# arnfred/Fast-Match

Measured on AMD Instinct MI355X. Metric: descriptor-pair distances/sec (cross-checked 1-NN + ratio test at 0.7), higher is better.
Workload: dtype int8

## Files before the change

fast-match_amd/csrc/filter6.hip:

```cpp
#include "tile_ops.h"
#include "fp6_filter.h"
#include "fp6_plan.h"

namespace fm {

typedef int   v8i_6  __attribute__((ext_vector_type(8)));
typedef int   v2i_6  __attribute__((ext_vector_type(2)));
typedef float v4f_6  __attribute__((ext_vector_type(4)));
typedef float v16f_6 __attribute__((ext_vector_type(16)));

#define F6_LDS_PTR(p) ((__attribute__((address_space(3))) void*)(p))
#define F6_GLB_PTR(p) ((const __attribute__((address_space(1))) void*)(p))
#define F6_INLINE __attribute__((always_inline))

constexpr int kF6NC = 4, kF6NW = 8;
constexpr int kF6PieceRows = 512;
constexpr int kF6ChunkRows = 32 * kF6NC * kF6NW;
constexpr int kF6Units = kStageRows / kTileRows;
constexpr float kF6Never = 3.0e38f;
constexpr int kF6HitSlots = 128;
static_assert(kF6HitSlots >= 64 && kF6HitSlots % 64 == 0, "a block's ballot must fit an empty list; the flush copies 64 at a time");
static_assert(3 * kStageBytes + kF6NW * kF6HitSlots * 8 <= 65536, "the kernel's static LDS");

struct F6Params {
    const uint8_t* col_rows6;
    const int32_t* col_stat;
    int            ncols;
    int            ncols_pad;
    const uint8_t* red_rows6;
    const float*   red_aux6;
    const int32_t* red_max;
    int            nstages, nsplit, nchunks, stages_per_split, ncols_alloc;
    int            nsplit_f, stages_per_split_f;
    unsigned long long* partial;
    const unsigned* cut;
    uint2*         rec;
    unsigned       cap;
    unsigned*      cnt;
    const int8_t*  col_rows8;
    const int32_t* col_norm;
    const int8_t*  red_rows8;
    const int32_t* red_norm;
    int            nred;
};

struct F6Batch {
    F6Params p[kRRBatchMax];
    int      n;
    int      first_block[kRRBatchMax + 1];
};

__device__ __forceinline__ void f6_issue_stage(const uint8_t* red_rows6, const float* red_aux6, int stage, char* buf, int wave, int lane)
{
    const uint8_t* src_rows = red_rows6 + (size_t)stage * kStageRowBytes;
    const int slot = lane & 7;
    constexpr int kPieces = 16 / kF6NW;
#pragma unroll
    for (int i = 0; i < kPieces; ++i) {
        const int g   = wave * kPieces + i;
        const int row = g * 8 + (lane >> 3);
        const uint8_t* src = src_rows + (unsigned)(row * kDim + 16 * (slot ^ ((row >> 1) & 7)));
        __builtin_amdgcn_global_load_lds(F6_GLB_PTR(src), F6_LDS_PTR(buf + g * 1024), 16, 0, 0);
    }
    if (wave == kF6NW - 1) {
        const float* src = red_aux6 + (size_t)stage * (kStageAuxBytes / 4) + (unsigned)(lane * 4);
        __builtin_amdgcn_global_load_lds(F6_GLB_PTR(src), F6_LDS_PTR(buf + kStageRowBytes), 16, 0, 0);
    }
}

struct F6Unit {
    v8i_6  a[2];
    v16f_6 c;
};

__device__ __forceinline__ float f6_max16(const v16f_6& a)
{
    const float m0 = fmaxf(fmaxf(a[0], a[1]), a[2]);
    const float m1 = fmaxf(fmaxf(a[3], a[4]), a[5]);
    const float m2 = fmaxf(fmaxf(a[6], a[7]), a[8]);
    const float m3 = fmaxf(fmaxf(a[9], a[10]), a[11]);
    const float m4 = fmaxf(fmaxf(a[12], a[13]), a[14]);
    const float m5 = fmaxf(fmaxf(m0, m1), m2);
    const float m6 = fmaxf(fmaxf(m3, m4), a[15]);
    return fmaxf(m5, m6);
}

__global__ __launch_bounds__(64 * kF6NW, 2)
void filter6_kernel(F6Batch b)
{
    __shared__ __attribute__((aligned(16))) char smem[3 * kStageBytes + kF6NW * kF6HitSlots * 8];
    int pair = 0;
#pragma unroll
    for (int i = 1; i < kRRBatchMax; ++i) pair += (int)blockIdx.x >= b.first_block[i] ? 1 : 0;
    const F6Params& p = b.p[pair];
    const int bid = (int)blockIdx.x - b.first_block[pair];

    const int tid  = threadIdx.x;
    const int lane = tid & 63;
    const int wave = tid >> 6;
    const int r32  = lane & 31;
    const int hs   = lane >> 5;
    const int nsplit = p.nsplit_f, nstages = p.nstages, per = p.stages_per_split_f, ncols = p.ncols, ncols_pad = p.ncols_pad;
    const int ncols_alloc = p.ncols_alloc;
    const int nch = (p.nchunks + 1) >> 1;
    const uint8_t* const red_rows6 = p.red_rows6;
    const float* const red_aux6 = p.red_aux6;
    uint2* const rec = p.rec;
    unsigned* const cnt = p.cnt;
    const unsigned cap = p.cap;
    const int split = __builtin_amdgcn_readfirstlane(bid / nch), chunk = bid - split * nch;
    if (split >= nsplit) return;
    const int st0 = split * per;
    const int st1 = min(st0 + per, nstages);
    const int cb  = chunk * kF6ChunkRows + wave * (32 * kF6NC);

    const unsigned dstar = *p.cut;
    if (dstar == kNoRatioCut) {
        if (tid == 0) cnt[1] = 1u;
        return;
    }
    {
        const int nslices = p.nsplit;
        const bool second = chunk * kF6ChunkRows + kF6PieceRows < ncols_alloc;
        for (int s = split; s < nslices; s += nsplit) {
            unsigned long long* mine = p.partial + (size_t)s * ncols_alloc + chunk * kF6ChunkRows;
            mine[tid] = ~0ull;
            if (second) mine[kF6PieceRows + tid] = ~0ull;
        }
    }

    v8i_6 bf[kF6NC][2];
    float thr[kF6NC];
    constexpr int kDmaPerWave = 16 / kF6NW;
    {
        const int um = p.red_max[0], em = p.red_max[1];
        v4i lo[kF6NC][2], stat[kF6NC];
        v2i_6 hi[kF6NC][2];
#pragma unroll
        for (int j = 0; j < kF6NC; ++j) {
            const int n = min(cb + 32 * j + r32, ncols_pad - 1);
#pragma unroll
            for (int h = 0; h < 2; ++h) {
                const uint8_t* src = p.col_rows6 + (size_t)n * kDim + 32 * (2 * h + hs);
                asm volatile("global_load_dwordx4 %0, %1, off" : "=v"(lo[j][h]) : "v"(src) : "memory");
                asm volatile("global_load_dwordx2 %0, %1, off offset:16" : "=v"(hi[j][h]) : "v"(src) : "memory");
            }
            asm volatile("global_load_dwordx4 %0, %1, off" : "=v"(stat[j]) : "v"(p.col_stat + 4 * (size_t)n) : "memory");
        }
        const int nfirst = min(st1 - st0, 2);
        if (nfirst > 0) f6_issue_stage(red_rows6, red_aux6, st0, smem, wave, lane);
        if (nfirst > 1) f6_issue_stage(red_rows6, red_aux6, st0 + 1, smem + kStageBytes, wave, lane);
        if (nfirst > 1) {
            if (wave == kF6NW - 1) asm volatile("s_waitcnt vmcnt(%0)" :: "n"(2 * (kDmaPerWave + 1)) : "memory");
            else                   asm volatile("s_waitcnt vmcnt(%0)" :: "n"(2 * kDmaPerWave) : "memory");
        } else {
            asm volatile("s_waitcnt vmcnt(0)" ::: "memory");
        }
#pragma unroll
        for (int j = 0; j < kF6NC; ++j)
            asm volatile("" : "+v"(lo[j][0]), "+v"(hi[j][0]), "+v"(lo[j][1]), "+v"(hi[j][1]), "+v"(stat[j]));
#pragma unroll
        for (int j = 0; j < kF6NC; ++j)
            if (cb + 32 * j + r32 >= ncols_pad) {
                lo[j][0] = lo[j][1] = v4i{0, 0, 0, 0};
                hi[j][0] = hi[j][1] = v2i_6{0, 0};
            }
#pragma unroll
        for (int j = 0; j < kF6NC; ++j) {
            const int n = cb + 32 * j + r32;
            thr[j] = n < ncols ? fp6_threshold_acc(fp6_threshold(stat[j][0], stat[j][1], stat[j][2], um, em, dstar)) : kF6Never;
#pragma unroll
            for (int h = 0; h < 2; ++h)
                bf[j][h] = v8i_6{lo[j][h][0], lo[j][h][1], lo[j][h][2], lo[j][h][3], hi[j][h][0], hi[j][h][1], 0, 0};
        }
    }

    const int sw = (r32 >> 1) & 7;
    int aoff0[2], aoff1[2];
#pragma unroll
    for (int h = 0; h < 2; ++h) {
        aoff0[h] = r32 * kDim + 16 * ((2 * (2 * h + hs)) ^ sw);
        aoff1[h] = r32 * kDim + 16 * ((2 * (2 * h + hs) + 1) ^ sw);
    }
    const int xoff = kStageRowBytes + 16 * hs;

    auto hand_over = [&](auto buf_tag, int st) F6_INLINE {
        constexpr int BUF = decltype(buf_tag)::value;
        if (st + 1 < st1) {
            if (wave == kF6NW - 1) asm volatile("s_waitcnt vmcnt(%0)" :: "n"(kDmaPerWave + 1) : "memory");
            else                   asm volatile("s_waitcnt vmcnt(%0)" :: "n"(kDmaPerWave) : "memory");
        } else {
            asm volatile("s_waitcnt vmcnt(0)" ::: "memory");
        }
        asm volatile("s_waitcnt lgkmcnt(0)\n\ts_barrier" ::: "memory");
        if (st + 2 < st1) f6_issue_stage(red_rows6, red_aux6, st + 2, smem + ((BUF + 2) % 3) * kStageBytes, wave, lane);
    };

    auto read_unit = [&](F6Unit& x, const char* buf, int u) F6_INLINE {
        const char* rows = buf + 32 * u * kDim;
#pragma unroll
        for (int h = 0; h < 2; ++h) {
            const v4i   lo = *(const v4i*)(rows + aoff0[h]);
            const v2i_6 hi = *(const v2i_6*)(rows + aoff1[h]);
            x.a[h] = __builtin_shufflevector(__builtin_shufflevector(lo, lo, 0, 1, 2, 3, -1, -1, -1, -1),
                                             __builtin_shufflevector(hi, hi, 0, 1, -1, -1, -1, -1, -1, -1), 0, 1, 2, 3, 8, 9, -1, -1);
        }
        v4f_6 c[4];
#pragma unroll
        for (int q = 0; q < 4; ++q) c[q] = *(const v4f_6*)(buf + xoff + (32 * u + 8 * q) * 4);
        x.c = v16f_6{c[0][0], c[0][1], c[0][2], c[0][3], c[1][0], c[1][1], c[1][2], c[1][3],
                     c[2][0], c[2][1], c[2][2], c[2][3], c[3][0], c[3][1], c[3][2], c[3][3]};
    };

    const uint2* const hits = (const uint2*)(smem + 3 * kStageBytes) + wave * kF6HitSlots;
    const unsigned hits_lds = (unsigned)(uintptr_t)F6_LDS_PTR(hits);
    unsigned nrec = 0;
    auto flush = [&]() F6_INLINE {
        unsigned base = 0;
        if (lane == 0) base = atomicAdd(cnt, nrec);
        base = (unsigned)__builtin_amdgcn_readfirstlane((int)base);
#pragma unroll
        for (int k = 0; k < kF6HitSlots / 64; ++k) {
            const unsigned i = (unsigned)(64 * k + lane);
            if (i < nrec) {
                const uint2 r = hits[i];
                if (base + i < cap) rec[base + i] = r;
                else                cnt[1] = 1u;
            }
        }
        asm volatile("s_waitcnt vmcnt(0)" ::: "memory");
        nrec = 0;
    };

    auto multiply = [&](const F6Unit& x, unsigned unit, F6Unit& y, const char* ybuf, auto yu_tag) F6_INLINE {
        v16f_6 acc[kF6NC];
        __builtin_amdgcn_s_setprio(2);
#pragma unroll
        for (int h = 0; h < 2; ++h)
#pragma unroll
            for (int j = 0; j < kF6NC; ++j)
                acc[j] = __builtin_amdgcn_mfma_scale_f32_32x32x64_f8f6f4(x.a[h], bf[j][h], h == 0 ? x.c : acc[j], 2, 2, 0, 0, 0, 0);
        __builtin_amdgcn_sched_barrier(0);
        if constexpr (decltype(yu_tag)::value >= 0) read_unit(y, ybuf, decltype(yu_tag)::value);
        __builtin_amdgcn_s_setprio(0);
        float tmax[kF6NC];
        bool any = false;
#pragma unroll
        for (int j = 0; j < kF6NC; ++j) {
            tmax[j] = f6_max16(acc[j]);
            any |= tmax[j] >= thr[j];
        }
        if (__builtin_amdgcn_ballot_w64(any) != 0ull) {
#pragma unroll
            for (int j = 0; j < kF6NC; ++j) {
                const bool hit = tmax[j] >= thr[j];
                const unsigned long long m = __builtin_amdgcn_ballot_w64(hit);
                if (m == 0ull) continue;
                const unsigned pc = (unsigned)__popcll(m);
                if (nrec + pc > (unsigned)kF6HitSlots) flush();
                const unsigned rank = __builtin_amdgcn_mbcnt_hi((unsigned)(m >> 32), __builtin_amdgcn_mbcnt_lo((unsigned)m, 0u));
                if (hit) {
                    const unsigned long long r = ((unsigned long long)(unit | ((unsigned)hs << 31)) << 32) | (unsigned)(cb + 32 * j + r32);
                    asm volatile("ds_write_b64 %0, %1" :: "v"(hits_lds + 8u * (nrec + rank)), "v"(r) : "memory");
                }
                nrec += pc;
            }
        }
    };

    F6Unit ua, ub;
    ub.a[0] = ub.a[1] = v8i_6{0, 0, 0, 0, 0, 0, 0, 0};
#pragma unroll
    for (int r = 0; r < 16; ++r) ub.c[r] = kFp6PadInit;
    std::integral_constant<int, 0> u0;  std::integral_constant<int, 1> u1;  std::integral_constant<int, 2> u2;
    std::integral_constant<int, 3> u3;  std::integral_constant<int, -1> none;
    auto stage = [&](auto buf_tag, int st) F6_INLINE {
        constexpr int BUF = decltype(buf_tag)::value;
        const char* buf = smem + BUF * kStageBytes;
        const unsigned unit0 = (unsigned)(st * kF6Units);
        hand_over(buf_tag, st);
        multiply(ub, unit0 - 1, ua, buf, u0);
        multiply(ua, unit0,     ub, buf, u1);
        multiply(ub, unit0 + 1, ua, buf, u2);
        multiply(ua, unit0 + 2, ub, buf, u3);
    };

    if (st0 >= st1) return;
    for (int st = st0; st < st1; st += 3) {
        stage(std::integral_constant<int, 0>{}, st);
        if (st + 1 < st1) stage(std::integral_constant<int, 1>{}, st + 1);
        if (st + 2 < st1) stage(std::integral_constant<int, 2>{}, st + 2);
    }
    multiply(ub, (unsigned)(st1 * kF6Units) - 1u, ua, smem, none);
    if (nrec != 0u) flush();
}

__global__ __launch_bounds__(256)
void rescore6_kernel(F6Batch b)
{
    const int lane = threadIdx.x & 63;
    const unsigned wave = (blockIdx.x * 256u + threadIdx.x) >> 6, nwaves = gridDim.x * 4u;
    for (int pi = 0; pi < b.n; ++pi) {
        const F6Params& p = b.p[pi];
        if (p.cnt[1] != 0u) continue;
        unsigned n = p.cnt[0];
        n = n < p.cap ? n : p.cap;
        const unsigned dstar = *p.cut;
        for (unsigned r = wave; r < n; r += nwaves) {
            const uint2 rc = p.rec[r];
            const int c = (int)rc.x;
            const int rr = lane & 15, kq = lane >> 4;
            const int m = (int)((rc.y & 0x7fffffffu) * 32u) + (rr & 3) + 8 * (rr >> 2) + 4 * (int)(rc.y >> 31);
            const int8_t* a = p.col_rows8 + (size_t)c * kDim + 32 * kq;
            const int8_t* y = p.red_rows8 + (size_t)m * kDim + 32 * kq;
            int dot = 0;
#pragma unroll
            for (int w = 0; w < 2; ++w) {
                const v4i x = *(const v4i*)(a + 16 * w);
                const v4i z = *(const v4i*)(y + 16 * w);
#pragma unroll
                for (int k = 0; k < 4; ++k) dot = __builtin_amdgcn_sdot4(x[k], z[k], dot, false);
            }
            dot += __shfl_xor(dot, 16);
            dot += __shfl_xor(dot, 32);
            const unsigned d2 = (unsigned)(p.col_norm[c] + p.red_norm[m] - 2 * dot);
            unsigned long long key = (m < p.nred && d2 < dstar) ? ((unsigned long long)d2 << 32) | (unsigned)m : ~0ull;
#pragma unroll
            for (int o = 8; o > 0; o >>= 1) {
                const unsigned long long other = __shfl_xor(key, o);
                key = other < key ? other : key;
            }
            if (lane == 0 && key != ~0ull) atomicMin(p.partial + c, key);
        }
    }
}

__global__ __launch_bounds__(256)
void prep6_kernel(const int8_t* __restrict__ rows8, int64_t n, int64_t n_pad, uint8_t* __restrict__ rows6,
                  float* __restrict__ aux6, int32_t* __restrict__ stat6, int32_t* __restrict__ max6)
{
    __shared__ uint8_t code[256];
    code[threadIdx.x] = (uint8_t)fp6_code((int)threadIdx.x);
    __syncthreads();
    const int k = threadIdx.x & 3;
    int umax = 0, emax = 0;
    for (int64_t row = (int64_t)blockIdx.x * 64 + (threadIdx.x >> 2); row < n_pad; row += (int64_t)gridDim.x * 64) {
        unsigned w[8] = {0, 0, 0, 0, 0, 0, 0, 0};
        int usq = 0, hsq = 0, esq = 0;
        if (row < n) {
            const uint4 lo = *(const uint4*)(rows8 + row * kDim + 32 * k), hi = *(const uint4*)(rows8 + row * kDim + 32 * k + 16);
            const unsigned src[8] = {lo.x, lo.y, lo.z, lo.w, hi.x, hi.y, hi.z, hi.w};
            unsigned long long bits = 0;
            int have = 0, out = 0;
#pragma unroll
            for (int i = 0; i < 32; ++i) {
                const int v = (int)(((src[i >> 2] >> (8 * (i & 3))) & 0xffu) ^ 0x80u);
                const int cd = code[v], x = fp6_value32(cd);
                usq += v * v; hsq += x * x; esq += (v - x) * (v - x);
                bits |= (unsigned long long)cd << have;
                have += 6;
                if (have >= 32) { w[out++] = (unsigned)bits; bits >>= 32; have -= 32; }
            }
        }
        *(uint4*)(rows6 + row * kDim + 32 * k)      = make_uint4(w[0], w[1], w[2], w[3]);
        *(uint4*)(rows6 + row * kDim + 32 * k + 16) = make_uint4(w[4], w[5], w[6], w[7]);
        usq += __shfl_xor(usq, 1); usq += __shfl_xor(usq, 2);
        hsq += __shfl_xor(hsq, 1); hsq += __shfl_xor(hsq, 2);
        esq += __shfl_xor(esq, 1); esq += __shfl_xor(esq, 2);
        if (k == 0) {
            *(int4*)(stat6 + 4 * row) = make_int4(usq, hsq, esq, 0);
            const int64_t st = row / kStageRows, r = row % kStageRows;
            aux6[st * 256 + r] = row < n ? fp6_acc_init(usq) : kFp6PadInit;
            aux6[st * 256 + 128 + r] = 0.f;
        }
        umax = max(umax, usq);
        emax = max(emax, esq);
    }
    for (int o = 32; o > 0; o >>= 1) {
        umax = max(umax, __shfl_xor(umax, o));
        emax = max(emax, __shfl_xor(emax, o));
    }
    if ((threadIdx.x & 63) == 0) {
        if (umax > 0) atomicMax(max6, umax);
        if (emax > 0) atomicMax(max6 + 1, emax);
    }
}

hipError_t launch_prep6(const Bank& b, int grid_max, hipStream_t stream)
{
    hipError_t e = hipMemsetAsync(b.max6, 0, 8, stream);
    if (e != hipSuccess) return e;
    int64_t grid = (b.n_pad + 63) / 64;
    if (grid_max > 0 && grid > grid_max) grid = grid_max;
    hipLaunchKernelGGL(prep6_kernel, dim3((unsigned)grid), dim3(256), 0, stream, (const int8_t*)b.rows8, b.n, b.n_pad,
                       b.rows6, b.aux6, b.stat6, b.max6);
    return hipGetLastError();
}

bool filter6_usable(const Bank& cols, const Bank& red)
{
    return cols.kind == FM_BANK_I8 && red.kind == FM_BANK_I8 && cols.dim == kDim && red.dim == kDim &&
           cols.rows6 && red.rows6 && cols.rows8 && red.rows8;
}

hipError_t launch_filter6(int n, const Bank* const* cols, const Bank* const* red, const RowReducePlan* plans,
                          unsigned long long* const* partial, const unsigned* const* cut, const Filter6Ws& ws, hipStream_t stream)
{
    if (n < 1 || n > kRRBatchMax) return hipErrorInvalidValue;
    uint2* const rec = ws.rec;  const unsigned cap = ws.cap;  unsigned* const cnt = ws.cnt;
    F6Batch b;
    long long total = 0;
    Fp6PlanPair pp[kRRBatchMax];
    for (int i = 0; i < n; ++i) pp[i] = Fp6PlanPair{(plans[i].nchunks + 1) / 2, (int)(red[i]->n_pad / kStageRows)};
    const int L = ws.nsplit == 0 ? fp6_plan_stages(pp, n, ws.resident, kFp6PlanOverhead) : 0;
    for (int i = 0; i < n; ++i) {
        const RowReducePlan& pl = plans[i];
        if (pl.nb != 4 || pl.nw != 8 || !filter6_usable(*cols[i], *red[i]) || !cut[i]) return hipErrorInvalidValue;
        F6Params& p = b.p[i];
        p.col_rows6 = cols[i]->rows6;  p.col_stat = cols[i]->stat6;  p.ncols = (int)cols[i]->n;  p.ncols_pad = (int)cols[i]->n_pad;
        p.red_rows6 = red[i]->rows6;   p.red_aux6 = red[i]->aux6;    p.red_max = red[i]->max6;
        p.nstages = (int)(red[i]->n_pad / kStageRows);
        p.nsplit = pl.nsplit;  p.nchunks = pl.nchunks;  p.stages_per_split = pl.stages_per_split;  p.ncols_alloc = pl.ncols_alloc;
        if (ws.nsplit < 0)      { p.nsplit_f = pl.nsplit;  p.stages_per_split_f = pl.stages_per_split; }
        else if (ws.nsplit > 0) fp6_plan_split_forced(p.nstages, ws.nsplit, &p.nsplit_f, &p.stages_per_split_f);
        else                    fp6_plan_split(p.nstages, L, &p.nsplit_f, &p.stages_per_split_f);
        p.partial = partial[i];  p.cut = cut[i];
        p.rec = rec + (size_t)i * cap;  p.cap = cap;  p.cnt = cnt + 2 * i;
        p.col_rows8 = cols[i]->rows8;  p.col_norm = cols[i]->norm;  p.red_rows8 = red[i]->rows8;  p.red_norm = red[i]->norm;
        p.nred = (int)red[i]->n;
        b.first_block[i] = (int)total;
        total += (long long)((pl.nchunks + 1) / 2) * p.nsplit_f;
    }
    if (total > INT32_MAX) return hipErrorInvalidValue;
    for (int i = n; i < kRRBatchMax; ++i) b.p[i] = b.p[0];
    b.first_block[n] = (int)total;
    for (int i = n + 1; i <= kRRBatchMax; ++i) b.first_block[i] = INT32_MAX;
    b.n = n;
    hipError_t e = hipMemsetAsync(cnt, 0, (size_t)n * 8, stream);
    if (e != hipSuccess) return e;
    hipLaunchKernelGGL(filter6_kernel, dim3((unsigned)total), dim3(64 * kF6NW), 0, stream, b);
    if ((e = hipGetLastError()) != hipSuccess) return e;
    hipStream_t tail = stream;
    if (ws.side) {
        if ((e = hipEventRecord(ws.ev_sweep, stream)) != hipSuccess || (e = hipStreamWaitEvent(ws.side, ws.ev_sweep, 0)) != hipSuccess) return e;
        tail = ws.side;
    }
    hipLaunchKernelGGL(rescore6_kernel, dim3(1024), dim3(256), 0, tail, b);
    return hipGetLastError();
}

}
```

fast-match_amd/csrc/fp6_filter.h:

```cpp
#pragma once
#include "ratio_cut.h"

namespace fm {

FM_HD inline int fp6_value32(int code)
{
    const int e = (code >> 3) & 3, mant = code & 7;
    return e == 0 ? 4 * mant : (8 + mant) << (e + 1);
}

FM_HD inline int fp6_code(int v)
{
    int best = 0, err = v;
    for (int c = 1; c < 32; ++c) {
        const int x = fp6_value32(c), e = x > v ? x - v : v - x;
        if (e < err) { best = c; err = e; }
    }
    return best;
}

FM_HD inline float fp6_acc_init(int usq) { return -(float)(usq >> 5) * (1.0f / 64.0f); }
constexpr float kFp6PadInit = -3.4e38f;

FM_HD inline double fp6_error_bound(int hatsq_c, int errsq_c, int usq_max_m, int errsq_max_m)
{
    const double e = sqrt((double)errsq_c) * sqrt((double)usq_max_m) + sqrt((double)hatsq_c) * sqrt((double)errsq_max_m);
    return e * (1.0 + 1.0 / 1048576.0) + 1.0 / 1024.0;
}

FM_HD inline double fp6_threshold(int usq_c, int hatsq_c, int errsq_c, int usq_max_m, int errsq_max_m, uint32_t dstar)
{
    return floor(((double)usq_c - (double)dstar + 1.0) * 0.5 - fp6_error_bound(hatsq_c, errsq_c, usq_max_m, errsq_max_m));
}

FM_HD inline float fp6_threshold_acc(double t)
{
    const double x = t * (1.0 / 1024.0);
    float f = (float)x;
    if ((double)f > x) f = nextafterf(f, -INFINITY);
    return f;
}

}
```

Before: 18890 billion.

## Screen fp6 MFMA tiles with per-stage max bias, apply per-row bias only on hits

The MFMA accumulators now start from zero instead of loading per-row bias vectors from LDS for every unit. A per-column screen threshold (thr minus the stage's maximum row bias, rounded downward) rejects tiles cheaply. The exact per-row bias is added only for column groups that pass the screen. The prep kernel is reorganised to process whole stages per block, so it can compute the per-stage minimum norm into the aux slot, and the aux data moves to a separate 4-slot LDS ring. This removes LDS reads and register pressure from the hot loop but adds extra work on screen hits, plus a mode-register rounding trick.

Result: faster. 19550 billion (median of 6 runs) (+3.5%).

```diff
diff --git a/fast-match_amd/csrc/filter6.hip b/fast-match_amd/csrc/filter6.hip
--- a/fast-match_amd/csrc/filter6.hip
+++ b/fast-match_amd/csrc/filter6.hip
@@ -17,10 +17,14 @@
 constexpr int kF6PieceRows = 512;
 constexpr int kF6ChunkRows = 32 * kF6NC * kF6NW;
 constexpr int kF6Units = kStageRows / kTileRows;
-constexpr float kF6Never = 3.0e38f;
 constexpr int kF6HitSlots = 128;
 static_assert(kF6HitSlots >= 64 && kF6HitSlots % 64 == 0, "a block's ballot must fit an empty list; the flush copies 64 at a time");
-static_assert(3 * kStageBytes + kF6NW * kF6HitSlots * 8 <= 65536, "the kernel's static LDS");
+constexpr int kF6RingSlots = 4;
+constexpr int kF6RingOff = 3 * kStageRowBytes;
+constexpr int kF6HitsOff = kF6RingOff + kF6RingSlots * kStageAuxBytes;
+constexpr int kF6LdsBytes = kF6HitsOff + kF6NW * kF6HitSlots * 8;
+constexpr int kF6SmaxWord = kStageRows;
+static_assert(kF6LdsBytes == 61440 && kF6LdsBytes <= 65536, "the kernel's static LDS");
 
 struct F6Params {
     const uint8_t* col_rows6;
@@ -50,7 +54,7 @@
     int      first_block[kRRBatchMax + 1];
 };
 
-__device__ __forceinline__ void f6_issue_stage(const uint8_t* red_rows6, const float* red_aux6, int stage, char* buf, int wave, int lane)
+__device__ __forceinline__ void f6_issue_stage(const uint8_t* red_rows6, const float* red_aux6, int stage, char* buf, char* aux, int wave, int lane)
 {
     const uint8_t* src_rows = red_rows6 + (size_t)stage * kStageRowBytes;
     const int slot = lane & 7;
@@ -64,13 +68,12 @@
     }
     if (wave == kF6NW - 1) {
         const float* src = red_aux6 + (size_t)stage * (kStageAuxBytes / 4) + (unsigned)(lane * 4);
-        __builtin_amdgcn_global_load_lds(F6_GLB_PTR(src), F6_LDS_PTR(buf + kStageRowBytes), 16, 0, 0);
+        __builtin_amdgcn_global_load_lds(F6_GLB_PTR(src), F6_LDS_PTR(aux), 16, 0, 0);
     }
 }
 
 struct F6Unit {
     v8i_6  a[2];
-    v16f_6 c;
 };
 
 __device__ __forceinline__ float f6_max16(const v16f_6& a)
@@ -88,7 +91,7 @@
 __global__ __launch_bounds__(64 * kF6NW, 2)
 void filter6_kernel(F6Batch b)
 {
-    __shared__ __attribute__((aligned(16))) char smem[3 * kStageBytes + kF6NW * kF6HitSlots * 8];
+    __shared__ __attribute__((aligned(16))) char smem[kF6LdsBytes];
     int pair = 0;
 #pragma unroll
     for (int i = 1; i < kRRBatchMax; ++i) pair += (int)blockIdx.x >= b.first_block[i] ? 1 : 0;
@@ -148,8 +151,8 @@
             asm volatile("global_load_dwordx4 %0, %1, off" : "=v"(stat[j]) : "v"(p.col_stat + 4 * (size_t)n) : "memory");
         }
         const int nfirst = min(st1 - st0, 2);
-        if (nfirst > 0) f6_issue_stage(red_rows6, red_aux6, st0, smem, wave, lane);
-        if (nfirst > 1) f6_issue_stage(red_rows6, red_aux6, st0 + 1, smem + kStageBytes, wave, lane);
+        if (nfirst > 0) f6_issue_stage(red_rows6, red_aux6, st0, smem, smem + kF6RingOff + (st0 & 3) * kStageAuxBytes, wave, lane);
+        if (nfirst > 1) f6_issue_stage(red_rows6, red_aux6, st0 + 1, smem + kStageRowBytes, smem + kF6RingOff + ((st0 + 1) & 3) * kStageAuxBytes, wave, lane);
         if (nfirst > 1) {
             if (wave == kF6NW - 1) asm volatile("s_waitcnt vmcnt(%0)" :: "n"(2 * (kDmaPerWave + 1)) : "memory");
             else                   asm volatile("s_waitcnt vmcnt(%0)" :: "n"(2 * kDmaPerWave) : "memory");
@@ -182,7 +185,6 @@
         aoff0[h] = r32 * kDim + 16 * ((2 * (2 * h + hs)) ^ sw);
         aoff1[h] = r32 * kDim + 16 * ((2 * (2 * h + hs) + 1) ^ sw);
     }
-    const int xoff = kStageRowBytes + 16 * hs;
 
     auto hand_over = [&](auto buf_tag, int st) F6_INLINE {
         constexpr int BUF = decltype(buf_tag)::value;
@@ -193,7 +195,8 @@
             asm volatile("s_waitcnt vmcnt(0)" ::: "memory");
         }
         asm volatile("s_waitcnt lgkmcnt(0)\n\ts_barrier" ::: "memory");
-        if (st + 2 < st1) f6_issue_stage(red_rows6, red_aux6, st + 2, smem + ((BUF + 2) % 3) * kStageBytes, wave, lane);
+        if (st + 2 < st1)
+            f6_issue_stage(red_rows6, red_aux6, st + 2, smem + ((BUF + 2) % 3) * kStageRowBytes, smem + kF6RingOff + ((st + 2) & 3) * kStageAuxBytes, wave, lane);
     };
 
     auto read_unit = [&](F6Unit& x, const char* buf, int u) F6_INLINE {
@@ -205,14 +208,9 @@
             x.a[h] = __builtin_shufflevector(__builtin_shufflevector(lo, lo, 0, 1, 2, 3, -1, -1, -1, -1),
                                              __builtin_shufflevector(hi, hi, 0, 1, -1, -1, -1, -1, -1, -1), 0, 1, 2, 3, 8, 9, -1, -1);
         }
-        v4f_6 c[4];
-#pragma unroll
-        for (int q = 0; q < 4; ++q) c[q] = *(const v4f_6*)(buf + xoff + (32 * u + 8 * q) * 4);
-        x.c = v16f_6{c[0][0], c[0][1], c[0][2], c[0][3], c[1][0], c[1][1], c[1][2], c[1][3],
-                     c[2][0], c[2][1], c[2][2], c[2][3], c[3][0], c[3][1], c[3][2], c[3][3]};
     };
 
-    const uint2* const hits = (const uint2*)(smem + 3 * kStageBytes) + wave * kF6HitSlots;
+    const uint2* const hits = (const uint2*)(smem + kF6HitsOff) + wave * kF6HitSlots;
     const unsigned hits_lds = (unsigned)(uintptr_t)F6_LDS_PTR(hits);
     unsigned nrec = 0;
     auto flush = [&]() F6_INLINE {
@@ -232,28 +230,42 @@
         nrec = 0;
     };
 
-    auto multiply = [&](const F6Unit& x, unsigned unit, F6Unit& y, const char* ybuf, auto yu_tag) F6_INLINE {
+    float thr_s[kF6NC];
+#pragma unroll
+    for (int j = 0; j < kF6NC; ++j) thr_s[j] = kF6Never;
+    auto multiply = [&](const F6Unit& x, unsigned unit, int xs, F6Unit& y, const char* ybuf, auto yu_tag, auto smax_tag, int smax_off) F6_INLINE {
         v16f_6 acc[kF6NC];
+        const v16f_6 zero = {0.f, 0.f, 0.f, 0.f, 0.f, 0.f, 0.f, 0.f, 0.f, 0.f, 0.f, 0.f, 0.f, 0.f, 0.f, 0.f};
         __builtin_amdgcn_s_setprio(2);
 #pragma unroll
         for (int h = 0; h < 2; ++h)
 #pragma unroll
             for (int j = 0; j < kF6NC; ++j)
-                acc[j] = __builtin_amdgcn_mfma_scale_f32_32x32x64_f8f6f4(x.a[h], bf[j][h], h == 0 ? x.c : acc[j], 2, 2, 0, 0, 0, 0);
+                acc[j] = __builtin_amdgcn_mfma_scale_f32_32x32x64_f8f6f4(x.a[h], bf[j][h], h == 0 ? zero : acc[j], 2, 2, 0, 0, 0, 0);
         __builtin_amdgcn_sched_barrier(0);
         if constexpr (decltype(yu_tag)::value >= 0) read_unit(y, ybuf, decltype(yu_tag)::value);
+        float smax = 0.f;
+        if constexpr (decltype(smax_tag)::value) smax = *(const float*)(smem + smax_off);
         __builtin_amdgcn_s_setprio(0);
         float tmax[kF6NC];
         bool any = false;
 #pragma unroll
         for (int j = 0; j < kF6NC; ++j) {
             tmax[j] = f6_max16(acc[j]);
-            any |= tmax[j] >= thr[j];
+            any |= tmax[j] >= thr_s[j];
         }
         if (__builtin_amdgcn_ballot_w64(any) != 0ull) {
 #pragma unroll
             for (int j = 0; j < kF6NC; ++j) {
-                const bool hit = tmax[j] >= thr[j];
+                if (__builtin_amdgcn_ballot_w64(tmax[j] >= thr_s[j]) == 0ull) continue;
+                float emax = kFp6PadInit;
+#pragma unroll
+                for (int q = 0; q < 4; ++q) {
+                    const v4f_6 s = *(const v4f_6*)(smem + xs + 16 * hs + 32 * q);
+#pragma unroll
+                    for (int k = 0; k < 4; ++k) emax = fmaxf(emax, acc[j][4 * q + k] + s[k]);
+                }
+                const bool hit = emax >= thr[j];
                 const unsigned long long m = __builtin_amdgcn_ballot_w64(hit);
                 if (m == 0ull) continue;
                 const unsigned pc = (unsigned)__popcll(m);
@@ -266,23 +278,27 @@
                 nrec += pc;
             }
         }
+        if constexpr (decltype(smax_tag)::value) {
+#pragma unroll
+            for (int j = 0; j < kF6NC; ++j) thr_s[j] = fp6_screen_threshold(thr[j], smax);
+        }
     };
 
     F6Unit ua, ub;
     ub.a[0] = ub.a[1] = v8i_6{0, 0, 0, 0, 0, 0, 0, 0};
-#pragma unroll
-    for (int r = 0; r < 16; ++r) ub.c[r] = kFp6PadInit;
     std::integral_constant<int, 0> u0;  std::integral_constant<int, 1> u1;  std::integral_constant<int, 2> u2;
     std::integral_constant<int, 3> u3;  std::integral_constant<int, -1> none;
+    std::true_type with_smax;  std::false_type no_smax;
     auto stage = [&](auto buf_tag, int st) F6_INLINE {
         constexpr int BUF = decltype(buf_tag)::value;
-        const char* buf = smem + BUF * kStageBytes;
+        const char* buf = smem + BUF * kStageRowBytes;
         const unsigned unit0 = (unsigned)(st * kF6Units);
+        const int xs = kF6RingOff + (st & 3) * kStageAuxBytes, xs_prev = kF6RingOff + ((st - 1) & 3) * kStageAuxBytes + 3 * 128;
         hand_over(buf_tag, st);
-        multiply(ub, unit0 - 1, ua, buf, u0);
-        multiply(ua, unit0,     ub, buf, u1);
-        multiply(ub, unit0 + 1, ua, buf, u2);
-        multiply(ua, unit0 + 2, ub, buf, u3);
+        multiply(ub, unit0 - 1, xs_prev,  ua, buf, u0, with_smax, xs + 4 * kF6SmaxWord);
+        multiply(ua, unit0,     xs,       ub, buf, u1, no_smax, 0);
+        multiply(ub, unit0 + 1, xs + 128, ua, buf, u2, no_smax, 0);
+        multiply(ua, unit0 + 2, xs + 256, ub, buf, u3, no_smax, 0);
     };
 
     if (st0 >= st1) return;
@@ -291,7 +307,7 @@
         if (st + 1 < st1) stage(std::integral_constant<int, 1>{}, st + 1);
         if (st + 2 < st1) stage(std::integral_constant<int, 2>{}, st + 2);
     }
-    multiply(ub, (unsigned)(st1 * kF6Units) - 1u, ua, smem, none);
+    multiply(ub, (unsigned)(st1 * kF6Units) - 1u, kF6RingOff + ((st1 - 1) & 3) * kStageAuxBytes + 3 * 128, ua, smem, none, no_smax, 0);
     if (nrec != 0u) flush();
 }
 
@@ -342,9 +358,14 @@
     __shared__ uint8_t code[256];
     code[threadIdx.x] = (uint8_t)fp6_code((int)threadIdx.x);
     __syncthreads();
+    __shared__ int stage_min[4];
     const int k = threadIdx.x & 3;
     int umax = 0, emax = 0;
-    for (int64_t row = (int64_t)blockIdx.x * 64 + (threadIdx.x >> 2); row < n_pad; row += (int64_t)gridDim.x * 64) {
+    int smin = INT32_MAX;
+    for (int64_t i = 0; ; ++i) {
+        const int64_t st = (i >> 1) * gridDim.x + blockIdx.x;
+        if (st >= n_pad / kStageRows) break;
+        const int64_t row = st * kStageRows + (i & 1) * 64 + (threadIdx.x >> 2);
         unsigned w[8] = {0, 0, 0, 0, 0, 0, 0, 0};
         int usq = 0, hsq = 0, esq = 0;
         if (row < n) {
@@ -369,12 +390,24 @@
         esq += __shfl_xor(esq, 1); esq += __shfl_xor(esq, 2);
         if (k == 0) {
             *(int4*)(stat6 + 4 * row) = make_int4(usq, hsq, esq, 0);
-            const int64_t st = row / kStageRows, r = row % kStageRows;
+            const int64_t r = row % kStageRows;
             aux6[st * 256 + r] = row < n ? fp6_acc_init(usq) : kFp6PadInit;
-            aux6[st * 256 + 128 + r] = 0.f;
+            if (r != 0) aux6[st * 256 + kStageRows + r] = 0.f;
         }
         umax = max(umax, usq);
         emax = max(emax, esq);
+        if (row < n) smin = min(smin, usq);
+        if (i & 1) {
+            for (int o = 32; o > 0; o >>= 1) smin = min(smin, __shfl_xor(smin, o));
+            if ((threadIdx.x & 63) == 0) stage_min[threadIdx.x >> 6] = smin;
+            __syncthreads();
+            if (threadIdx.x == 0) {
+                const int m = min(min(stage_min[0], stage_min[1]), min(stage_min[2], stage_min[3]));
+                aux6[st * 256 + kStageRows] = m != INT32_MAX ? fp6_acc_init(m) : kFp6PadInit;
+            }
+            __syncthreads();
+            smin = INT32_MAX;
+        }
     }
     for (int o = 32; o > 0; o >>= 1) {
         umax = max(umax, __shfl_xor(umax, o));
@@ -390,7 +423,7 @@
 {
     hipError_t e = hipMemsetAsync(b.max6, 0, 8, stream);
     if (e != hipSuccess) return e;
-    int64_t grid = (b.n_pad + 63) / 64;
+    int64_t grid = b.n_pad / kStageRows;
     if (grid_max > 0 && grid > grid_max) grid = grid_max;
     hipLaunchKernelGGL(prep6_kernel, dim3((unsigned)grid), dim3(256), 0, stream, (const int8_t*)b.rows8, b.n, b.n_pad,
                        b.rows6, b.aux6, b.stat6, b.max6);
diff --git a/fast-match_amd/csrc/fp6_filter.h b/fast-match_amd/csrc/fp6_filter.h
--- a/fast-match_amd/csrc/fp6_filter.h
+++ b/fast-match_amd/csrc/fp6_filter.h
@@ -21,6 +21,7 @@
 
 FM_HD inline float fp6_acc_init(int usq) { return -(float)(usq >> 5) * (1.0f / 64.0f); }
 constexpr float kFp6PadInit = -3.4e38f;
+constexpr float kF6Never = 3.0e38f;
 
 FM_HD inline double fp6_error_bound(int hatsq_c, int errsq_c, int usq_max_m, int errsq_max_m)
 {
@@ -41,4 +42,24 @@
     return f;
 }
 
+FM_HD inline float fp6_screen_threshold(float thr, float smax)
+{
+#if defined(__HIP_DEVICE_COMPILE__)
+    float d;
+    asm("s_setreg_imm32_b32 hwreg(HW_REG_MODE, 0, 2), 2\n\t"
+        "v_sub_f32 %0, %1, %2\n\t"
+        "s_nop 1\n\t"
+        "s_setreg_imm32_b32 hwreg(HW_REG_MODE, 0, 2), 0\n\t"
+        "s_nop 1" : "=v"(d) : "v"(thr), "v"(smax));
+    return d;
+#else
+    const volatile float s = thr - smax;
+    if (isinf(s)) return s > 0.f ? 3.402823466e38f : s;
+    const volatile float bb = s - thr;
+    const volatile float ra = thr - (s - bb), rb = -smax - bb;
+    const float err = ra + rb;
+    return err < 0.f ? nextafterf(s, -INFINITY) : s;
+#endif
 }
+
+}
```
